# jyakaranda/A-LeGO-LOAM

Hardware: AMD Instinct MI355X
Metric: scans/sec (16x1800 LiDAR) full IP->LO->LM loop (higher is better)
Workload: dtype f32/f64

## Files before the change

### a-lego-loam_amd/csrc/alego_api.hip

```cpp
#include <hip/hip_runtime.h>

#include <cmath>
#include <cstdio>
#include <cstdlib>
#include <algorithm>
#include <cstring>
#include <mutex>
#include <set>
#include <string>
#include <vector>

#include "../../include/alego_mi355x.h"
#include "dev_common.h"
#include "dev_mem.h"
#include "front_end.h"
#include "lm_ctx.h"
#include "lm_host.h"
#include "merge_math.h"
#include "thin_math.h"
#include "loop_ctx.h"
#include "pgraph.h"
#include "prof.h"
#include "reloc.h"
#include "stream_plan.h"
// ... 769 lines not shown
    prev = m.stamp;
    const double qw = m.orientation[0], qx = m.orientation[1], qy = m.orientation[2], qz = m.orientation[3];
    double roll, pitch, yaw;
    {
      const double dd = qx * qx + qy * qy + qz * qz + qw * qw, sc = 2.0 / dd;
      const double xs = qx * sc, ys = qy * sc, zs = qz * sc;
      const double wx = qw * xs, wy = qw * ys, wz = qw * zs, xx = qx * xs, xy = qx * ys, xz = qx * zs, yy = qy * ys, yz = qy * zs, zz = qz * zs;
      const double m00 = 1.0 - (yy + zz), m10 = xy + wz, m20 = xz - wy, m21 = yz + wx, m22 = 1.0 - (xx + yy);
      if (std::fabs(m20) >= 1) {
        yaw = 0;
        const double delta = std::atan2(m21, m22);
        if (m20 < 0) { pitch = M_PI / 2.0; roll = delta; } else { pitch = -M_PI / 2.0; roll = delta; }
      } else {
        pitch = -std::asin(m20);
        roll = std::atan2(m21 / std::cos(pitch), m22 / std::cos(pitch));
        yaw = std::atan2(m10 / std::cos(pitch), m00 / std::cos(pitch));
      }
    }
    const double acc_x = m.linear_acceleration[0] + 9.81 * std::sin(pitch);
    const double acc_y = m.linear_acceleration[1] - 9.81 * std::cos(pitch) * std::sin(roll);
    const double acc_z = m.linear_acceleration[2] - 9.81 * std::cos(pitch) * std::cos(roll);
    const float w = (float)qw, x = (float)qx, y = (float)qy, z = (float)qz;
    const float tx = 2 * x, ty = 2 * y, tz = 2 * z;
    const float twx = tx * w, twy = ty * w, twz = tz * w, txx = tx * x, txy = ty * x, txz = tz * x, tyy = ty * y, tyz = tz * y, tzz = tz * z;
    const float R[3][3] = {{1 - (tyy + tzz), txy - twz, txz + twy}, {txy + twz, 1 - (txx + tzz), tyz - twx}, {txz - twy, tyz + twx, 1 - (txx + tyy)}};
    const float a[3] = {(float)acc_x, (float)acc_y, (float)acc_z};
    double* o = &pre[(size_t)i * 7];
    o[0] = m.stamp; o[1] = roll; o[2] = pitch; o[3] = yaw;
    for (int k = 0; k < 3; ++k) o[4 + k] = (double)(R[k][0] * a[0] + (R[k][1] * a[1] + R[k][2] * a[2]));
  }
  DevPool T;
  double* dp;
  HIP_TRY(h, T.get(&dp, pre.size(), false));
  hipStream_t S = stream_of(h, slot);
  HIP_TRY(h, hipMemcpyAsync(dp, pre.data(), pre.size() * 8, hipMemcpyHostToDevice, S));
  launch_lo_imu_push(h->d, slot, dp, n, S);
  HIP_TRY(h, hipStreamSynchronize(S));
  h->imu_last_stamp[slot] = prev;
  return 0;
}

int alego_profile_enable(alego_handle* h, int on) {
  if (!h) return ALEGO_ERR_ARG;
  hipSetDevice(h->device);
  HIP_TRY(h, sync_all(h));
  h->prof.reset();
  h->prof.on = on != 0;
  return 0;
}

int alego_profile_report(alego_handle* h, char* names, int names_cap, double* total_ms, int* launches, int cap) {
  if (!h) return ALEGO_ERR_ARG;
  hipSetDevice(h->device);
  HIP_TRY(h, sync_all(h));
  Profiler& P = h->prof;
  const int nk = (int)P.names.size();
  std::vector<double> tot(nk, 0.0);
  std::vector<int> cnt(nk, 0);
  for (auto& r : P.recs) {
    float ms = 0.f;
    if (hipEventElapsedTime(&ms, r.a, r.b) == hipSuccess) { tot[r.id] += ms; cnt[r.id]++; }
  }
  std::string joined;
  for (int i = 0; i < nk; ++i) { if (i) joined += ";"; joined += P.names[i]; }
  if ((int)joined.size() + 1 > names_cap || nk > cap) { h->err = "profile_report: buffers too small"; return ALEGO_ERR_CAPACITY; }
  std::memcpy(names, joined.c_str(), joined.size() + 1);
  for (int i = 0; i < nk; ++i) { total_ms[i] = tot[i]; launches[i] = cnt[i]; }
  return nk;
}

int alego_debug_voxel(alego_handle* h, const alego_point* pts, int n, float leaf, alego_point* out, int cap) {
  if (!h || n < 0 || (n > 0 && !pts)) return ALEGO_ERR_ARG;
  hipSetDevice(h->device);
  g_prof = &h->prof;
  DevPool T;
  float4 *din = nullptr, *dout = nullptr;
  int* cnt = nullptr;
  const int c = n > 0 ? n : 1;
  HIP_TRY(h, T.get(&din, (size_t)c, false)); HIP_TRY(h, T.get(&dout, (size_t)c, false)); HIP_TRY(h, T.get(&cnt, 2, false));
  const int hc[2] = {n, 0};
  HIP_TRY(h, hipMemcpy(cnt, hc, 8, hipMemcpyHostToDevice));
  if (n) HIP_TRY(h, hipMemcpy(din, pts, (size_t)n * 16, hipMemcpyHostToDevice));
  VoxJob job{din, cnt, dout, cnt + 1, nullptr, leaf, c, c, nullptr, 0};
  VoxCtx V;
  if (vox_create(&V, &job, 1, &h->err)) return ALEGO_ERR_HIP;
  int rc = vox_run(V, h->stream, &h->err);
  hipError_t e = hipStreamSynchronize(h->stream);
  int nout = 0;
  if (e == hipSuccess) e = hipMemcpy(&nout, cnt + 1, 4, hipMemcpyDeviceToHost);
  if (e == hipSuccess && rc == 0 && nout > cap) { h->err = "debug_voxel: output capacity"; rc = ALEGO_ERR_CAPACITY; }
  if (e == hipSuccess && rc == 0 && nout) e = hipMemcpy(out, dout, (size_t)nout * 16, hipMemcpyDeviceToHost);
  vox_destroy(&V);
  if (e != hipSuccess) { h->err = std::string("debug_voxel: ") + hipGetErrorString(e); return ALEGO_ERR_HIP; }
  return rc ? rc : nout;
}

int alego_debug_math(alego_handle* h, int mode, const float* a, const float* b, float* out, int n) {
  if (!h || n < 0 || mode < 0 || mode > 3 || (n > 0 && (!a || !out || (mode < 2 && !b)))) return ALEGO_ERR_ARG;
  if (n == 0) return 0;
  hipSetDevice(h->device);
  DevPool T;
  float *da, *db, *dout;
  HIP_TRY(h, T.get(&da, (size_t)n, false)); HIP_TRY(h, T.get(&db, (size_t)n, false)); HIP_TRY(h, T.get(&dout, (size_t)n, false));
  HIP_TRY(h, hipMemcpy(da, a, (size_t)n * 4, hipMemcpyHostToDevice));
  if (b) HIP_TRY(h, hipMemcpy(db, b, (size_t)n * 4, hipMemcpyHostToDevice));
  launch_atan2f_probe(da, db, dout, n, mode, h->stream);
  HIP_TRY(h, hipStreamSynchronize(h->stream));
  HIP_TRY(h, hipMemcpy(out, dout, (size_t)n * 4, hipMemcpyDeviceToHost));
  return 0;
}
int alego_debug_atan2f(alego_handle* h, const float* y, const float* x, float* out, int n) { return alego_debug_math(h, 0, y, x, out, n); }

int alego_debug_std_sort(alego_handle* h, const uint32_t* keys, int n, int depth_limit, int32_t* order) {
  if (!h || n < 0 || n > 4096 || (n > 0 && (!keys || !order))) return ALEGO_ERR_ARG;
  if (n == 0) return 0;
  hipSetDevice(h->device);
  DevPool T;
  uint32_t* dk;
  int* dp;
  HIP_TRY(h, T.get(&dk, (size_t)n, false)); HIP_TRY(h, T.get(&dp, (size_t)n, false));
  HIP_TRY(h, hipMemcpy(dk, keys, (size_t)n * 4, hipMemcpyHostToDevice));
  if (launch_stdsort_probe(dk, n, depth_limit, dp, h->stream)) return ALEGO_ERR_ARG;
  HIP_TRY(h, hipStreamSynchronize(h->stream));
  std::vector<int> pos(n), arr(n);
  HIP_TRY(h, hipMemcpy(pos.data(), dp, (size_t)n * 4, hipMemcpyDeviceToHost));
  for (int i = 0; i < n; ++i) { if (pos[i] < 0 || pos[i] >= n) { h->err = "alego_debug_std_sort: arrangement out of range"; return ALEGO_ERR_HIP; } arr[pos[i]] = i; }
  std::stable_sort(arr.begin(), arr.end(), [&](int a, int b) { return keys[a] < keys[b]; });
  for (int i = 0; i < n; ++i) order[i] = arr[i];
  return 0;
}

int alego_debug_eval_blocks(alego_handle* h, int type, int n, const double* geom13, const double* params6, double* res, double* jac6) {
  if (!h || n < 0 || type < 0 || type > 3 || !params6 || (n > 0 && (!geom13 || !res || !jac6))) return ALEGO_ERR_ARG;
  if (n == 0) return 0;
  hipSetDevice(h->device);
  DevPool T;
  double *dg, *dp, *dr, *dj;
  HIP_TRY(h, T.get(&dg, (size_t)n * 13, false)); HIP_TRY(h, T.get(&dp, 6, false)); HIP_TRY(h, T.get(&dr, (size_t)n, false)); HIP_TRY(h, T.get(&dj, (size_t)n * 6, false));
  HIP_TRY(h, hipMemcpy(dg, geom13, (size_t)n * 13 * 8, hipMemcpyHostToDevice));
  HIP_TRY(h, hipMemcpy(dp, params6, 48, hipMemcpyHostToDevice));
  launch_dbg_eval_blocks(type, n, dg, dp, dr, dj, h->stream);
  HIP_TRY(h, hipStreamSynchronize(h->stream));
  HIP_TRY(h, hipMemcpy(res, dr, (size_t)n * 8, hipMemcpyDeviceToHost));
  HIP_TRY(h, hipMemcpy(jac6, dj, (size_t)n * 48, hipMemcpyDeviceToHost));
  return 0;
}

int alego_debug_transform_to_start(alego_handle* h, const double* params6, const alego_point* pts, int n, alego_point* out) {
  if (!h || n < 0 || !params6 || (n > 0 && (!pts || !out))) return ALEGO_ERR_ARG;
  if (n == 0) return 0;
  hipSetDevice(h->device);
  DevPool T;
  double* dp;
  float4 *di, *dout;
  HIP_TRY(h, T.get(&dp, 6, false)); HIP_TRY(h, T.get(&di, (size_t)n, false)); HIP_TRY(h, T.get(&dout, (size_t)n, false));
  HIP_TRY(h, hipMemcpy(dp, params6, 48, hipMemcpyHostToDevice));
  HIP_TRY(h, hipMemcpy(di, pts, (size_t)n * 16, hipMemcpyHostToDevice));
  launch_dbg_transform_to_start(dp, di, n, dout, h->stream);
  HIP_TRY(h, hipStreamSynchronize(h->stream));
  HIP_TRY(h, hipMemcpy(out, dout, (size_t)n * 16, hipMemcpyDeviceToHost));
  return 0;
}

int alego_debug_check_guards(char* report, int cap) {
  std::string r;
  const int bad = guard_check(&r);
// ... 651 lines not shown
```

### a-lego-loam_amd/csrc/kernels_voxel.hip

```cpp
#include <algorithm>
#include <cstring>

#include <hip/hip_runtime.h>

#include <vector>

#include "voxel.h"
#include "wave.h"
#include "vgrid.h"
#include "dev_mem.h"
#include "prof.h"

typedef unsigned long long u64;

__device__ __forceinline__ bool vx_enabled(const VoxJob& J) { return J.enable == nullptr || *J.enable != 0; }

#ifndef VX_SMALL_MAX
#define VX_SMALL_MAX 8192
#endif

#ifndef VG_T
#define VG_T 512
#endif
#define VG_W (VG_T / 64)
// ... 154 lines not shown
  __threadfence_block();
  __syncthreads();
  VG_TICK(11);
  if (J.mode == 1) {
    for (int i = tid; i < min(n, J.out_cap); i += VG_T) outp[i] = J.in[(unsigned)srt[i]];
    if (tid == 0) { *J.n_out = min(n, J.out_cap); if (n > J.out_cap && J.overflow) *J.overflow = 1;
                    if (J.n_sel_out) J.n_sel_out[(size_t)sel * J.n_sel_stride] = min(n, J.out_cap); }
    __syncthreads();
    return;
  }
  auto head_rounds = [&](int r0, bool* head) {
    u64 cur[VG_U], prv[VG_U];
#pragma unroll
    for (int k = 0; k < VG_U; ++k) {
      const int i = r0 + 64 * k + lane;
      cur[k] = srt[min(i, n - 1)]; prv[k] = srt[max(min(i, n - 1) - 1, 0)];
    }
#pragma unroll
    for (int k = 0; k < VG_U; ++k) {
      const int i = r0 + 64 * k + lane;
      head[k] = i < seg1 && (i == 0 || (unsigned)(cur[k] >> 32) != (unsigned)(prv[k] >> 32));
    }
  };
  int* hl = reinterpret_cast<int*>(keys);
  int heads = 0;
  for (int r0 = seg0; r0 < seg1; r0 += 64 * VG_U) {
    bool head[VG_U];
    head_rounds(r0, head);
#pragma unroll
    for (int k = 0; k < VG_U; ++k) {
      const u64 hb = __ballot(head[k]);
      if (head[k]) hl[seg0 + heads + (int)__builtin_amdgcn_mbcnt_hi((unsigned)(hb >> 32), __builtin_amdgcn_mbcnt_lo((unsigned)hb, 0u))] = r0 + 64 * k + lane;
      heads += (int)__popcll(hb);
    }
  }
  if (lane == 0) s_w[wave] = heads;
  __threadfence_block();
  __syncthreads();
  if (tid == 0) {
    int run = 0;
    for (int w = 0; w < VG_W; ++w) { s_wbase[w] = run; run += s_w[w]; }
    s_wbase[VG_W] = run;
    int nf = n;
    s_nextfirst[VG_W] = n;
    for (int w = VG_W - 1; w >= 0; --w) { if (s_w[w] > 0) nf = hl[min(n, w * seglen)]; s_nextfirst[w] = nf; }
  }
  __syncthreads();
  const int nvox = s_wbase[VG_W];
  VG_TICK(12);
  for (int r = tid; r < min(nvox, J.out_cap); r += VG_T) {
    int w = 0;
#pragma unroll
    for (int q = 1; q < VG_W; ++q) w += (r >= s_wbase[q]) ? 1 : 0;
    const int loc = r - s_wbase[w], ws0 = min(n, w * seglen);
    const int a = hl[ws0 + loc], bn = hl[ws0 + min(loc + 1, s_w[w] - 1)];
    const int b = loc + 1 < s_w[w] ? bn : s_nextfirst[w + 1];
    float sx = 0.f, sy = 0.f, sz = 0.f, si = 0.f;
    for (int j = a; j < b; j += 8) {
      unsigned q[8];
      float4 pt[8];
#pragma unroll
      for (int k = 0; k < 8; ++k) q[k] = (unsigned)srt[min(j + k, b - 1)];
#pragma unroll
      for (int k = 0; k < 8; ++k) pt[k] = J.in[q[k]];
#pragma unroll
      for (int k = 0; k < 8; ++k) if (j + k < b) { sx += pt[k].x; sy += pt[k].y; sz += pt[k].z; si += pt[k].w; }
    }
    const float fn = (float)(b - a);
    J.out[r] = make_float4(sx / fn, sy / fn, sz / fn, si / fn);
  }
  if (tid == 0) { *J.n_out = min(nvox, J.out_cap); if (nvox > J.out_cap && J.overflow) *J.overflow = 1; }
  __syncthreads();
  VG_TICK(13);
}
#ifdef ALEGO_TIMING
extern "C" void alego_vg_times(long long* out) { (void)hipMemcpyFromSymbol(out, HIP_SYMBOL(vg_times), sizeof(long long) * 16); }
#endif

#define VX_SB 512
#define VS_W (VX_SB / 64)
#define VS_DMAX 9
#define VS_ND (1 << VS_DMAX)
__device__ __forceinline__ bool vx_less(const unsigned* key, unsigned a, unsigned b) { return key[a] < key[b] || (key[a] == key[b] && a < b); }

__device__ void vox_small_job(const VoxCtx& V, int job) {
  const VoxJob J = V.jobs[job];
  const int n = min(*J.n_in, J.cap);
  const int tid = threadIdx.x, lane = tid & 63, wave = tid >> 6;
  extern __shared__ __attribute__((aligned(16))) unsigned char vs_smem[];
  unsigned* s_key = reinterpret_cast<unsigned*>(vs_smem);
  unsigned short* s_ia = reinterpret_cast<unsigned short*>(vs_smem + 4 * VX_SMALL_MAX);
  unsigned short* s_ib = reinterpret_cast<unsigned short*>(vs_smem + 6 * VX_SMALL_MAX);
  unsigned short* s_cnt = reinterpret_cast<unsigned short*>(vs_smem + 8 * VX_SMALL_MAX);
  __shared__ float s_red[6][VX_SB / 64];
  __shared__ int s_scan[VX_SB / 64];
  __shared__ int s_tot[VS_ND];
  const int sel = (J.mode == 1 && J.out_sel) ? *J.out_sel : 0;
  float4* const outp = J.out + (size_t)sel * (J.mode == 1 ? J.out_stride : 0);
  if (n == 0) { if (tid == 0) { *J.n_out = 0; if (J.mode == 1 && J.n_sel_out) J.n_sel_out[(size_t)sel * J.n_sel_stride] = 0; } return; }
  const float inv = 1.0f / J.leaf;
  VG_TICK(0);
  float mn[3] = {3.402823466e+38f, 3.402823466e+38f, 3.402823466e+38f}, mx[3] = {-3.402823466e+38f, -3.402823466e+38f, -3.402823466e+38f};
  for (int i = tid; i < n; i += VX_SB) vgr_box_add(mn, mx, J.in[i]);
#pragma unroll
  for (int a = 0; a < 3; ++a) {
    bfly_minmax_f32(mn[a], mx[a]);
    if (lane == 0) { s_red[a][wave] = mn[a]; s_red[3 + a][wave] = mx[a]; }
  }
  __syncthreads();
#pragma unroll
  for (int a = 0; a < 3; ++a) {
    mn[a] = s_red[a][0]; mx[a] = s_red[3 + a][0];
#pragma unroll
    for (int w = 1; w < VX_SB / 64; ++w) { mn[a] = fminf(mn[a], s_red[a][w]); mx[a] = fmaxf(mx[a], s_red[3 + a][w]); }
  }
  if (tid < 3) {
    unsigned* bb = V.bbox + job * 8;
    bb[tid] = vgr_enc(tid == 0 ? mn[0] : tid == 1 ? mn[1] : mn[2]);
    bb[4 + tid] = ~vgr_enc(tid == 0 ? mx[0] : tid == 1 ? mx[1] : mx[2]);
  }
  if (J.mode == 1 && tid < 6 && J.box_out) J.box_out[(size_t)sel * 8 + (tid < 3 ? tid : tid + 1)] = tid == 0 ? mn[0] : tid == 1 ? mn[1] : tid == 2 ? mn[2] : tid == 3 ? mx[0] : tid == 4 ? mx[1] : mx[2];
  if (vgr_leaf_too_small(mn, mx, inv)) {
    for (int i = tid; i < min(n, J.out_cap); i += VX_SB) outp[i] = J.in[i];
    if (tid == 0) { *J.n_out = min(n, J.out_cap); if (n > J.out_cap && J.overflow) *J.overflow = 1;
                    if (J.mode == 1 && J.n_sel_out) J.n_sel_out[(size_t)sel * J.n_sel_stride] = min(n, J.out_cap); }
    return;
  }
  VG_TICK(1);
  const VgrGeom g = vgr_geom(mn, mx, inv);
  for (int i = tid; i < n; i += VX_SB) s_key[i] = vgr_id(g, J.in[i], inv);
  VG_TICK(2);
  const int bits = max(vgr_bits(g.T), 1);
  const int P = (bits + VS_DMAX - 1) / VS_DMAX, D = (bits + P - 1) / P, nd = 1 << D;
  const unsigned dmask = (unsigned)(nd - 1);
  const int seglen = ((n + VX_SB - 1) / VX_SB) * 64;
  const int seg0 = min(n, wave * seglen), seg1 = min(n, seg0 + seglen);
  unsigned short* my = s_cnt + wave * VS_ND;
  for (int p = 0; p < P; ++p) {
    const unsigned short* src = (p & 1) ? s_ia : s_ib;
    unsigned short* dst = (p & 1) ? s_ib : s_ia;
    const int sh = p * D;
    __syncthreads();
    for (int q = lane; q < nd; q += 64) my[q] = 0;
    for (int sweep = 0; sweep < 2; ++sweep) {
      if (sweep == 1) {
        __syncthreads();
        if (tid < nd) {
          int run = 0;
#pragma unroll
          for (int w = 0; w < VS_W; ++w) { const int c = s_cnt[w * VS_ND + tid]; s_cnt[w * VS_ND + tid] = (unsigned short)run; run += c; }
          s_tot[tid] = run;
        }
        __syncthreads();
        if (wave == 0) {
          constexpr int PER = VS_ND / 64;
          int v[PER], sum = 0;
#pragma unroll
          for (int k = 0; k < PER; ++k) { const int dgt = lane * PER + k; v[k] = dgt < nd ? s_tot[dgt] : 0; sum += v[k]; }
          const int incl = wave_incl_scan(sum);
          int run = incl - sum;
#pragma unroll
          for (int k = 0; k < PER; ++k) { const int dgt = lane * PER + k; if (dgt < nd) s_tot[dgt] = run; run += v[k]; }
        }
        __syncthreads();
      }
      for (int r0 = seg0; r0 < seg1; r0 += 64) {
        const int i = r0 + lane;
        const bool valid = i < seg1;
        const unsigned idx = valid ? (p == 0 ? (unsigned)i : (unsigned)src[i]) : 0u;
        const unsigned dg = valid ? (s_key[idx] >> sh) & dmask : 0u;
        unsigned long long m = __ballot(valid);
        for (int bit = 0; bit < D; ++bit) {
          const bool one = (dg >> bit) & 1u;
          const unsigned long long bal = __ballot(one);
          m &= one ? bal : ~bal;
        }
        const int rank = (int)__builtin_amdgcn_mbcnt_hi((unsigned)(m >> 32), __builtin_amdgcn_mbcnt_lo((unsigned)m, 0u));
        if (sweep == 1 && valid) dst[(int)my[dg] + s_tot[dg] + rank] = (unsigned short)idx;
        if (valid && rank == 0) my[dg] = (unsigned short)(my[dg] + (int)__popcll(m));
      }
    }
  }
  __syncthreads();
  const unsigned short* srt = (P & 1) ? s_ia : s_ib;
  unsigned short* hl = (P & 1) ? s_ib : s_ia;
  VG_TICK(3);
  if (J.mode == 1) {
    for (int i = tid; i < min(n, J.out_cap); i += VX_SB) outp[i] = J.in[srt[i]];
    if (tid == 0) { *J.n_out = min(n, J.out_cap); if (n > J.out_cap && J.overflow) *J.overflow = 1;
                    if (J.n_sel_out) J.n_sel_out[(size_t)sel * J.n_sel_stride] = min(n, J.out_cap); }
    __syncthreads();
    return;
  }
  int heads = 0;
  for (int r0 = seg0; r0 < seg1; r0 += 64) {
    const int i = r0 + lane;
    const bool head = i < seg1 && (i == 0 || s_key[srt[i]] != s_key[srt[i - 1]]);
    heads += (int)__popcll(__ballot(head));
  }
  if (lane == 0) s_scan[wave] = heads;
  __syncthreads();
  int vbase = 0, nvox = 0;
#pragma unroll
  for (int w = 0; w < VX_SB / 64; ++w) { const int c = s_scan[w]; if (w < wave) vbase += c; nvox += c; }
  for (int r0 = seg0; r0 < seg1; r0 += 64) {
    const int i = r0 + lane;
    const bool head = i < seg1 && (i == 0 || s_key[srt[i]] != s_key[srt[i - 1]]);
    const unsigned long long hb = __ballot(head);
    if (head) hl[vbase + (int)__builtin_amdgcn_mbcnt_hi((unsigned)(hb >> 32), __builtin_amdgcn_mbcnt_lo((unsigned)hb, 0u))] = (unsigned short)i;
    vbase += (int)__popcll(hb);
  }
  __syncthreads();
  VG_TICK(4);
  VG_TICK(5);
  VG_TICK(6);
  for (int r = tid; r < min(nvox, J.out_cap); r += VX_SB) {
    const int a = hl[r], b = r + 1 < nvox ? (int)hl[r + 1] : n;
    float sx = 0.f, sy = 0.f, sz = 0.f, si = 0.f;
    for (int j = a; j < b; j += 4) {
      float4 pt[4];
#pragma unroll
      for (int k = 0; k < 4; ++k) pt[k] = J.in[srt[min(j + k, b - 1)]];
#pragma unroll
      for (int k = 0; k < 4; ++k) if (j + k < b) { sx += pt[k].x; sy += pt[k].y; sz += pt[k].z; si += pt[k].w; }
    }
    const float fn = (float)(b - a);
    J.out[r] = make_float4(sx / fn, sy / fn, sz / fn, si / fn);
  }
  if (tid == 0) { *J.n_out = min(nvox, J.out_cap); if (nvox > J.out_cap && J.overflow) *J.overflow = 1; }
  __syncthreads();
  VG_TICK(7);
}
__global__ void __launch_bounds__(VX_SB) vox_small(VoxCtx V) {
  extern __shared__ __attribute__((aligned(16))) unsigned char vs_smem_k[];
  const int cnt = V.cnt[0];
  for (int j = blockIdx.x; j < cnt; j += gridDim.x) {
    vox_small_job(V, V.list_small[j]);
    __syncthreads();
  }
  const int nbig = V.cnt[1];
  if ((int)blockIdx.x < V.grid_big) {
    for (int j = blockIdx.x; j < nbig; j += min((int)gridDim.x, V.grid_big)) {
      vox_big_job(V, V.list_big[j], vs_smem_k);
      __syncthreads();
    }
  }
}

__global__ void __launch_bounds__(256) vox_plan(VoxCtx V) {
  __shared__ int s_n[2];
  if (threadIdx.x < 2) s_n[threadIdx.x] = 0;
  __syncthreads();
  for (int j = threadIdx.x; j < V.njobs; j += 256) {
    const VoxJob J = V.jobs[j];
    if (!vx_enabled(J)) continue;
    const int n = min(*J.n_in, J.cap);
    if (n == 0) { *J.n_out = 0; if (J.mode == 1 && J.n_sel_out) J.n_sel_out[(size_t)(J.out_sel ? *J.out_sel : 0) * J.n_sel_stride] = 0; continue; }
    if (n <= VX_SMALL_MAX) V.list_small[atomicAdd(&s_n[0], 1)] = j;
    else V.list_big[atomicAdd(&s_n[1], 1)] = j;
  }
  __syncthreads();
  if (threadIdx.x < 2) V.cnt[threadIdx.x] = s_n[threadIdx.x];
}

#define VX_SMALL_LDS (8 * VX_SMALL_MAX + 2 * VS_W * VS_ND)
int vox_create(VoxCtx* V, const VoxJob* jobs, int njobs, std::string* err) {
  std::memset(V, 0, sizeof(*V));
  if (hipFuncSetAttribute(reinterpret_cast<const void*>(vox_small), hipFuncAttributeMaxDynamicSharedMemorySize, VX_SMALL_LDS) != hipSuccess) { *err = "vox_create: hipFuncSetAttribute"; return -2; }
// ... 36 lines not shown
```

### a-lego-loam_amd/csrc/lm_host.hip

```cpp
#include "lm_host.h"
#include "dev_mem.h"

#include <cstdio>
#include <cstdlib>
#include <algorithm>
#include <cstring>
#include <vector>

#include <rccl/rccl.h>

#include "kf_store.h"
#include "voxel.h"
#include "gmap.h"
#include "loc_math.h"
#include "pgraph.h"
#include "merge.h"
#include "merge_math.h"
#include "thin.h"
#include "thin_math.h"

struct LmHost {
  alego_params P;
  int n_slots;
  int gsize;
// ... 46 lines not shown
  int* li = L.li + (size_t)slot * LI_COUNT;
  for (int m = 0; m < 2; ++m) {
    const int cap = m ? L.total_cap : L.kf_cap_c;
    VoxJob j{(m ? L.kf_tmp_s : L.kf_tmp_c) + (size_t)slot * cap, li + LI_TMPN_C + m, (m ? L.kfs_s : L.kfs_c) + kf_row_at(L, slot, 0) * cap, li + LI_SORT_N + m, li + LI_KF_PENDING,
             m ? P.lm_leaf_surf : P.lm_leaf_corner, cap, cap, li + LI_OVERFLOW, 0};
    j.mode = 1; j.out_sel = li + LI_KF_PEND_RING; j.out_stride = cap;
    j.box_out = L.kfs_box + kf_run_at(L, slot, m, 0) * 8; j.n_sel_out = L.kfs_n + kf_run_at(L, slot, m, 0); j.n_sel_stride = 1;
    out->push_back(j);
  }
}
}

LmHost* lm_host_create(const alego_params& P, const DevCtx& d, int n_slots, int gsize, const std::vector<hipStream_t>& st, std::string* err) {
  LmHost* lm = new LmHost();
  lm->P = P; lm->n_slots = n_slots; lm->gsize = gsize; lm->st = st; lm->frames.assign(n_slots, 0);
  lm->gv.small_max = gv_small_max_env();
  VoxCtx vz; std::memset(&vz, 0, sizeof(VoxCtx));
  lm->vm.assign(st.size(), vz); lm->v2.assign(st.size(), vz); lm->vk.assign(st.size(), vz);
  lm->work.assign(st.size(), MapWork{nullptr, nullptr, 0});
  LmCtx& L = lm->L;
  std::memset(&L, 0, sizeof(L));
  L.K = P.recent_keyframe_num > 0 ? P.recent_keyframe_num : 1;
  L.KR = L.K + 1;
  L.fr_stride = L.KR; L.fr_mod = L.KR;
  lm->fallback_ok = n_slots <= 64 || !d.opt_map_merge;
  L.in_cap_c = d.fcap[F_LSHARP]; L.in_cap_s = d.N; L.in_cap_o = d.N;
  L.kf_cap_c = d.fcap[F_LSHARP];
  L.kf_cap_s = P.kf_cap_surf > 0 ? std::min(P.kf_cap_surf, d.N) : d.N / 2;
  L.kf_cap_o = P.kf_cap_outlier > 0 ? std::min(P.kf_cap_outlier, d.N) : d.N / 4;
  L.kf_cap_s = std::max(L.kf_cap_s, L.kf_cap_c - L.kf_cap_o);
  L.total_cap = L.kf_cap_s + L.kf_cap_o;
  L.map_cap_c = L.K * L.kf_cap_c; L.map_cap_s = L.K * L.total_cap;
  L.gcap = n_slots <= 64 ? (1 << 20) : (1 << 18);
  L.qcap = L.kf_cap_c + L.total_cap;
  {
    const size_t mx = lm_solve_row_bytes_max();
    const char* e = getenv("ALEGO_LM_ROW_LDS");
    int dev = 0, cus = 256;
    if (hipGetDevice(&dev) != hipSuccess || hipDeviceGetAttribute(&cus, hipDeviceAttributeMultiprocessorCount, dev) != hipSuccess) cus = 256;
    const size_t dflt = gsize > cus ? (size_t)72 * 1024 : lm_solve_row_bytes_default();
    L.solve_row_bytes = (int)(e ? std::min(mx, (size_t)std::max(0, atoi(e))) : std::min(mx, dflt));
  }
  const size_t B = n_slots;
  bool ok = true;
  ok = ok && A(lm, &L.li, B * LI_COUNT, err) && A(lm, &L.ld, B * LD_COUNT, err);
  ok = ok && A(lm, &L.stage_odom, B * 2 * 8, err);
  ok = ok && A(lm, &L.in_corner, B * L.in_cap_c, err) && A(lm, &L.in_surf, B * L.in_cap_s, err) && A(lm, &L.in_outl, B * L.in_cap_o, err);
  ok = ok && ring_alloc(lm, L, B * L.KR, err);
  ok = ok && A(lm, &L.kf_tmp_c, B * L.kf_cap_c, err) && A(lm, &L.kf_tmp_s, B * L.total_cap, err);
  ok = ok && A(lm, &L.rec, B * L.K, err) && A(lm, &L.rec_prev, B * L.K, err);
  ok = ok && A(lm, &L.U_c, B * L.map_cap_c, err) && A(lm, &L.U_s, B * L.map_cap_s, err) && A(lm, &L.Ucnt_c, B * L.map_cap_c, err) && A(lm, &L.Ucnt_s, B * L.map_cap_s, err);
  ok = ok && A(lm, &L.newkeys, B * 2 * L.total_cap, err) && A(lm, &L.map_bbox, B * 2 * 8, err);
  {
    double* part = nullptr; int* ctl = nullptr; double* state = nullptr;
    ok = ok && A(lm, &part, B * 32, err) && A(lm, &ctl, B * 8, err) && A(lm, &state, B * 64, err);
    L.shard_part = part; L.shard_ctl = ctl; L.shard_state = state;
  }
  ok = ok && A(lm, &L.map_corner_raw, lm->fallback_ok ? B * L.map_cap_c : 1, err) && A(lm, &L.map_surf_raw, lm->fallback_ok ? B * L.map_cap_s : 1, err);
  ok = ok && A(lm, &L.map_corner_ds, B * L.map_cap_c, err) && A(lm, &L.map_surf_ds, B * L.map_cap_s, err);
  ok = ok && A(lm, &L.cur_corner_ds, B * L.kf_cap_c, err) && A(lm, &L.cur_surf_ds, B * L.kf_cap_s, err) && A(lm, &L.cur_outl_ds, B * L.kf_cap_o, err);
  ok = ok && A(lm, &L.cur_total, B * L.total_cap, err) && A(lm, &L.cur_total_ds, B * L.total_cap, err);
  ok = ok && A(lm, &L.grid, B * 2, err) && A(lm, &L.cell_start, B * 2 * ((size_t)L.gcap + 1), err) && A(lm, &L.cell_cur, B * 2 * ((size_t)L.gcap + 1), err);
  ok = ok && A(lm, &L.cell_pts, B * 2 * L.map_cap_s, err);
  ok = ok && A(lm, &L.blocks, B * L.qcap * 8, err) && A(lm, &L.crows, B * L.qcap * 10, err) && A(lm, &L.knn, B * L.qcap * 5, err);
  if (!ok) { lm_host_destroy(lm); return nullptr; }
  std::vector<double> ld(B * LD_COUNT, 0.0);
  for (size_t b = 0; b < B; ++b) { ld[b * LD_COUNT + LD_Q_M2O] = 1.0; ld[b * LD_COUNT + LD_Q_O2L] = 1.0; ld[b * LD_COUNT + LD_Q_M2L] = 1.0; }
  if (hipMemcpy(L.ld, ld.data(), ld.size() * sizeof(double), hipMemcpyHostToDevice) != hipSuccess) { *err = "lm_host_create: upload failed"; lm_host_destroy(lm); return nullptr; }
  std::vector<int> li0(B * LI_COUNT, 0);
  for (size_t b = 0; b < B; ++b) li0[b * LI_COUNT + LI_LATEST] = -1;
  if (hipMemcpy(L.li, li0.data(), li0.size() * sizeof(int), hipMemcpyHostToDevice) != hipSuccess) { *err = "lm_host_create: upload failed"; lm_host_destroy(lm); return nullptr; }
  for (size_t g = 0; g < st.size(); ++g) {
  std::vector<VoxJob> jm, j1, j2, jk;
  for (size_t b = g * gsize; b < B && b < (g + 1) * (size_t)gsize; ++b) {
    int* li = L.li + b * LI_COUNT;
    if (lm->fallback_ok) {
      jm.push_back(VoxJob{L.map_corner_raw + b * L.map_cap_c, li + LI_KRAW_C, L.map_corner_ds + b * L.map_cap_c, li + LI_KDS_C, li + LI_REBUILD_FB, P.lm_leaf_corner, L.map_cap_c, L.map_cap_c, li + LI_OVERFLOW, 0});
      jm.push_back(VoxJob{L.map_surf_raw + b * L.map_cap_s, li + LI_KRAW_S, L.map_surf_ds + b * L.map_cap_s, li + LI_KDS_S, li + LI_REBUILD_FB, P.lm_leaf_surf, L.map_cap_s, L.map_cap_s, li + LI_OVERFLOW, 0});
    }
    j1.push_back(VoxJob{L.in_corner + b * L.in_cap_c, li + LI_NIN_C, L.cur_corner_ds + b * L.kf_cap_c, li + LI_NCUR_C, li + LI_RUN, P.lm_leaf_corner, L.in_cap_c, L.kf_cap_c, li + LI_OVERFLOW, 0});
    j1.push_back(VoxJob{L.in_surf + b * L.in_cap_s, li + LI_NIN_S, L.cur_surf_ds + b * L.kf_cap_s, li + LI_NCUR_S, li + LI_RUN, P.lm_leaf_surf, L.in_cap_s, L.kf_cap_s, li + LI_OVERFLOW, 0});
    j1.push_back(VoxJob{L.in_outl + b * L.in_cap_o, li + LI_NIN_O, L.cur_outl_ds + b * L.kf_cap_o, li + LI_NCUR_O, li + LI_RUN, P.lm_leaf_outlier, L.in_cap_o, L.kf_cap_o, li + LI_OVERFLOW, 0});
    j2.push_back(VoxJob{L.cur_total + b * L.total_cap, li + LI_NTOTAL, L.cur_total_ds + b * L.total_cap, li + LI_NTOTAL_DS, li + LI_RUN, P.lm_leaf_surf, L.total_cap, L.total_cap, li + LI_OVERFLOW, 0});
    kf_sort_jobs(L, P, (int)b, &jk);
  }
  const int ns = (int)j1.size() / 3;
  jm.insert(jm.end(), j1.begin(), j1.end());
  jm.insert(jm.end(), jk.begin(), jk.end());
  if (vox_create(&lm->vm[g], jm.data(), (int)jm.size(), err) || vox_create(&lm->v2[g], j2.data(), (int)j2.size(), err) ||
      vox_create(&lm->vk[g], jk.data(), (int)jk.size(), err)) { lm_host_destroy(lm); return nullptr; }
  const bool big_scans = d.N > 8 * 8192;
  lm->vm[g].grid_small = 3 * ns + std::max(2, ns / 2);
  if (const char* e = getenv("ALEGO_VOX_GRID_DIV")) { const int dv = std::max(1, atoi(e)); lm->vm[g].grid_small = std::max(2, lm->vm[g].grid_small / dv); lm->v2[g].grid_small = std::max(1, lm->v2[g].grid_small / dv); }
  lm->vm[g].grid_big = (!d.opt_map_merge || big_scans) ? std::max(2, ns / 2) : std::min(8, std::max(2, ns / 2));
  lm->v2[g].grid_big = big_scans ? std::max(2, ns / 2) : std::max(1, ns / 16);
  lm->vk[g].grid_small = 2; lm->vk[g].grid_big = 2;
  MapWork& W = lm->work[g];
  W.cap = std::max(4096, 64 * ns);
  if (!A(lm, &W.items, (size_t)W.cap, err) || !A(lm, &W.count, 2, err)) { lm_host_destroy(lm); return nullptr; }
  }
  return lm;
}

void lm_host_destroy(LmHost* lm) {
  if (!lm) return;
  if (lm->comm) { (void)ncclCommDestroy(lm->comm); lm->comm = nullptr; }
  for (auto& v : lm->vm) vox_destroy(&v);
  for (auto& v : lm->v2) vox_destroy(&v);
  for (auto& v : lm->vk) vox_destroy(&v);
  if (lm->vloc_made) vox_destroy(&lm->vloc);
  gv_destroy(&lm->gv);
  lm->mg_pairs.clear(); lm->mg_items.clear(); lm->mg_tail.clear(); lm->mg_moves.clear();
  lm->th_jobs.clear(); lm->th_ints.clear(); lm->th_prot.clear(); lm->th_items.clear(); lm->th_pts.clear(); lm->th_rows.clear(); lm->th_pose.clear();
  lm->mem.clear();
  delete lm;
}

static bool dbg_sync(hipStream_t st, const char* what, std::string* err) {
  static const bool on = getenv("ALEGO_DEBUG_SYNC") != nullptr;
  if (!on) return true;
  hipError_t e = hipStreamSynchronize(st);
  if (e == hipSuccess) e = hipGetLastError();
  fprintf(stderr, "[alego dbg] %s: %s\n", what, hipGetErrorString(e));
  if (e != hipSuccess) { *err = std::string(what) + ": " + hipGetErrorString(e); return false; }
  return true;
}

static int map_sequence(LmHost* lm, const DevCtx& d, const LmCtx& L, int g, hipStream_t st, std::string* err) {
  if (!d.opt_map_merge) {
    if (!lm->fallback_ok) { *err = "ALEGO_MAP_MERGE=0 needs the handle to be created with it (more than 64 slots)"; return ALEGO_ERR_ARG; }
    launch_lm_concat(d, L, st);
    if (!dbg_sync(st, "lm_concat", err)) return ALEGO_ERR_HIP;
  }
  if (int r = vox_run(lm->vm[g], st, err)) return r;
  if (!dbg_sync(st, "vox round 1", err)) return ALEGO_ERR_HIP;
  launch_map_update(d, L, lm->work[g], st);
  if (!dbg_sync(st, "map_update", err)) return ALEGO_ERR_HIP;
  if (d.opt_map_merge) {
    launch_map_accum(d, L, lm->work[g], st);
    if (!dbg_sync(st, "map_accum", err)) return ALEGO_ERR_HIP;
  }
  launch_lm_grid(d, L, st);
  if (!dbg_sync(st, "lm_grid", err)) return ALEGO_ERR_HIP;
  return 0;
}

static int lm_allreduce(void* ctx, double* buf, size_t count, hipStream_t st) {
  LmHost* lm = static_cast<LmHost*>(ctx);
  const ncclResult_t r = ncclAllReduce(buf, buf, count, ncclDouble, ncclSum, lm->comm, st);
  if (r != ncclSuccess) { lm->dist_err = std::string("ncclAllReduce: ") + ncclGetErrorString(r); return ALEGO_ERR_HIP; }
  return 0;
}

struct LmAsync { hipStream_t front, back; hipEvent_t staged, back_same, back_other; long k; };
static int lm_sequence(LmHost* lm, const DevCtx& d, int stage, const std::vector<char>& odom_valid, std::string* err, hipStream_t st_override = nullptr, const LmAsync* A = nullptr) {
  const int g = d.slot0 / lm->gsize;
  hipStream_t st = A ? A->back : (st_override ? st_override : lm->st[g]);
  LmCtx L = lm->L;
  L.vox_bbox = lm->vm[g].bbox; L.vox_slot0 = g * lm->gsize;
  int n_run = 0, n_norun = 0;
  for (int i = 0; i < d.n_launch; ++i) {
    long& f = lm->frames[d.slot0 + i];
    const bool run = odom_valid[i] && (f % lm->P.lm_every) == 0;
    if (odom_valid[i]) ++f;
    run ? ++n_run : ++n_norun;
  }
// ... 826 lines not shown
```

### a-lego-loam_amd/csrc/voxel.h

```cpp
#ifndef ALEGO_VOXEL_H_
#define ALEGO_VOXEL_H_
#include <hip/hip_runtime.h>

#include <string>

struct VoxJob {
  const float4* in;
  const int* n_in;
  float4* out;
  int* n_out;
  const int* enable;
  float leaf;
  int cap;
  int out_cap;
  int* overflow;
  int off;
  int mode;
  const int* out_sel;
  int out_stride;
  float* box_out;
  int* n_sel_out;
  int n_sel_stride;
};

struct VoxCtx {
  VoxJob* jobs;
  int njobs;
  unsigned* bbox;
  unsigned* keys;
  unsigned long long *pairs_a, *pairs_b;
  int *list_small, *list_big, *cnt;
  int grid_small, grid_big;
  unsigned total;
};

int vox_create(VoxCtx* V, const VoxJob* jobs, int njobs, std::string* err);
void vox_destroy(VoxCtx* V);
int vox_run(const VoxCtx& V, hipStream_t st, std::string* err);

#endif
```

Before: 472,500.

## Add tiny-job wave path, presorted merge fast path, and atomic digit counting to voxel sort

Jobs with 64 or fewer points are handled by a single wavefront that ranks keys through readlane comparisons instead of a radix sort. For jobs flagged as presorted (the concatenated total cloud), the kernel counts descents and, when the keys are already sorted or form two sorted runs or a short unsorted tail, builds the permutation by binary-search merging and skips the radix passes. The radix histogram pass now uses packed 16-bit shared-memory atomics instead of the earlier counting loop. These paths add branches and a pass to detect descents, and the atomic counting may contend on heavily repeated digits.

```diff
diff --git a/a-lego-loam_amd/csrc/alego_api.hip b/a-lego-loam_amd/csrc/alego_api.hip
--- a/a-lego-loam_amd/csrc/alego_api.hip
+++ b/a-lego-loam_amd/csrc/alego_api.hip
@@ -875,6 +875,7 @@
   HIP_TRY(h, hipMemcpy(cnt, hc, 8, hipMemcpyHostToDevice));
   if (n) HIP_TRY(h, hipMemcpy(din, pts, (size_t)n * 16, hipMemcpyHostToDevice));
   VoxJob job{din, cnt, dout, cnt + 1, nullptr, leaf, c, c, nullptr, 0};
+  job.presorted_hint = 1;
   VoxCtx V;
   if (vox_create(&V, &job, 1, &h->err)) return ALEGO_ERR_HIP;
   int rc = vox_run(V, h->stream, &h->err);
diff --git a/a-lego-loam_amd/csrc/kernels_voxel.hip b/a-lego-loam_amd/csrc/kernels_voxel.hip
--- a/a-lego-loam_amd/csrc/kernels_voxel.hip
+++ b/a-lego-loam_amd/csrc/kernels_voxel.hip
@@ -260,6 +260,101 @@
 #define VS_DMAX 9
 #define VS_ND (1 << VS_DMAX)
 __device__ __forceinline__ bool vx_less(const unsigned* key, unsigned a, unsigned b) { return key[a] < key[b] || (key[a] == key[b] && a < b); }
+#ifndef VX_CNT_ATOMIC
+#define VX_CNT_ATOMIC 1
+#endif
+#ifndef VX_TINY
+#define VX_TINY 1
+#endif
+#ifndef VX_MERGE
+#define VX_MERGE 1
+#endif
+static_assert(VX_SMALL_MAX % VX_SB == 0 && VX_SMALL_MAX / VX_SB * 64 < 65536, "a wavefront's segment must fit a 16-bit digit counter");
+__device__ __forceinline__ void vx_wave_sync() {
+  __builtin_amdgcn_fence(__ATOMIC_RELEASE, "wavefront");
+  __builtin_amdgcn_wave_barrier();
+  __builtin_amdgcn_fence(__ATOMIC_ACQUIRE, "wavefront");
+}
+__device__ __forceinline__ int vx_count_below(const unsigned* k, int lo, int hi, unsigned key, bool or_equal) {
+  int a = lo, e = hi;
+  while (a < e) {
+    const int m = (a + e) >> 1;
+    const unsigned v = k[m];
+    if (or_equal ? v <= key : v < key) a = m + 1; else e = m;
+  }
+  return a - lo;
+}
+
+#if VX_TINY
+__device__ void vox_tiny_job(const VoxCtx& V, int job, const VoxJob& J, int n, unsigned* s_key, unsigned short* srt, unsigned short* hl) {
+  const int lane = threadIdx.x;
+  const bool valid = lane < n;
+  const int sel = (J.mode == 1 && J.out_sel) ? *J.out_sel : 0;
+  float4* const outp = J.out + (size_t)sel * (J.mode == 1 ? J.out_stride : 0);
+  const float inv = 1.0f / J.leaf;
+  VG_TICK(0);
+  float mn[3] = {3.402823466e+38f, 3.402823466e+38f, 3.402823466e+38f}, mx[3] = {-3.402823466e+38f, -3.402823466e+38f, -3.402823466e+38f};
+  const float4 pt = J.in[min(lane, n - 1)];
+  if (valid) vgr_box_add(mn, mx, pt);
+#pragma unroll
+  for (int a = 0; a < 3; ++a) bfly_minmax_f32(mn[a], mx[a]);
+  if (lane < 3) {
+    unsigned* bb = V.bbox + job * 8;
+    bb[lane] = vgr_enc(lane == 0 ? mn[0] : lane == 1 ? mn[1] : mn[2]);
+    bb[4 + lane] = ~vgr_enc(lane == 0 ? mx[0] : lane == 1 ? mx[1] : mx[2]);
+  }
+  if (J.mode == 1 && lane < 6 && J.box_out) J.box_out[(size_t)sel * 8 + (lane < 3 ? lane : lane + 1)] = lane == 0 ? mn[0] : lane == 1 ? mn[1] : lane == 2 ? mn[2] : lane == 3 ? mx[0] : lane == 4 ? mx[1] : mx[2];
+  if (vgr_leaf_too_small(mn, mx, inv)) {
+    if (lane < min(n, J.out_cap)) outp[lane] = pt;
+    if (lane == 0) { *J.n_out = min(n, J.out_cap); if (n > J.out_cap && J.overflow) *J.overflow = 1;
+                     if (J.mode == 1 && J.n_sel_out) J.n_sel_out[(size_t)sel * J.n_sel_stride] = min(n, J.out_cap); }
+    return;
+  }
+  VG_TICK(1);
+  const VgrGeom g = vgr_geom(mn, mx, inv);
+  const unsigned key = vgr_id(g, pt, inv);
+  if (valid) s_key[lane] = key;
+  VG_TICK(2);
+  int rank = 0;
+  for (int j = 0; j < n; ++j) {
+    const unsigned kj = (unsigned)__builtin_amdgcn_readlane((int)key, j);
+    rank += (kj < key || (kj == key && j < lane)) ? 1 : 0;
+  }
+  if (valid) srt[rank] = (unsigned short)lane;
+  vx_wave_sync();
+  VG_TICK(3);
+  if (J.mode == 1) {
+    if (lane < min(n, J.out_cap)) outp[lane] = J.in[srt[lane]];
+    if (lane == 0) { *J.n_out = min(n, J.out_cap); if (n > J.out_cap && J.overflow) *J.overflow = 1;
+                     if (J.n_sel_out) J.n_sel_out[(size_t)sel * J.n_sel_stride] = min(n, J.out_cap); }
+    return;
+  }
+  const bool head = valid && (lane == 0 || s_key[srt[lane]] != s_key[srt[lane - 1]]);
+  const unsigned long long hb = __ballot(head);
+  const int nvox = (int)__popcll(hb);
+  if (head) hl[(int)__builtin_amdgcn_mbcnt_hi((unsigned)(hb >> 32), __builtin_amdgcn_mbcnt_lo((unsigned)hb, 0u))] = (unsigned short)lane;
+  vx_wave_sync();
+  VG_TICK(4);
+  VG_TICK(5);
+  VG_TICK(6);
+  if (lane < min(nvox, J.out_cap)) {
+    const int r = lane;
+    const int a = hl[r], b = r + 1 < nvox ? (int)hl[r + 1] : n;
+    float sx = 0.f, sy = 0.f, sz = 0.f, si = 0.f;
+    for (int j = a; j < b; j += 4) {
+      float4 q[4];
+#pragma unroll
+      for (int k = 0; k < 4; ++k) q[k] = J.in[srt[min(j + k, b - 1)]];
+#pragma unroll
+      for (int k = 0; k < 4; ++k) if (j + k < b) { sx += q[k].x; sy += q[k].y; sz += q[k].z; si += q[k].w; }
+    }
+    const float fn = (float)(b - a);
+    J.out[r] = make_float4(sx / fn, sy / fn, sz / fn, si / fn);
+  }
+  if (lane == 0) { *J.n_out = min(nvox, J.out_cap); if (nvox > J.out_cap && J.overflow) *J.overflow = 1; }
+  VG_TICK(7);
+}
+#endif
 
 __device__ void vox_small_job(const VoxCtx& V, int job) {
   const VoxJob J = V.jobs[job];
@@ -273,9 +368,18 @@
   __shared__ float s_red[6][VX_SB / 64];
   __shared__ int s_scan[VX_SB / 64];
   __shared__ int s_tot[VS_ND];
+#if VX_MERGE
+  __shared__ int s_desc[2];
+#endif
   const int sel = (J.mode == 1 && J.out_sel) ? *J.out_sel : 0;
   float4* const outp = J.out + (size_t)sel * (J.mode == 1 ? J.out_stride : 0);
   if (n == 0) { if (tid == 0) { *J.n_out = 0; if (J.mode == 1 && J.n_sel_out) J.n_sel_out[(size_t)sel * J.n_sel_stride] = 0; } return; }
+#if VX_TINY
+  if (n <= 64) {
+    if (wave == 0) vox_tiny_job(V, job, J, n, s_key, s_ia, s_ib);
+    return;
+  }
+#endif
   const float inv = 1.0f / J.leaf;
   VG_TICK(0);
   float mn[3] = {3.402823466e+38f, 3.402823466e+38f, 3.402823466e+38f}, mx[3] = {-3.402823466e+38f, -3.402823466e+38f, -3.402823466e+38f};
@@ -306,15 +410,53 @@
   }
   VG_TICK(1);
   const VgrGeom g = vgr_geom(mn, mx, inv);
+#if VX_MERGE
+  if (J.presorted_hint && tid < 2) s_desc[tid] = tid ? n : 0;
+#endif
   for (int i = tid; i < n; i += VX_SB) s_key[i] = vgr_id(g, J.in[i], inv);
   VG_TICK(2);
+  bool sorted = false;
+#if VX_MERGE
+  if (J.presorted_hint) {
+    __syncthreads();
+    for (int i0 = 0; i0 < n; i0 += VX_SB) {
+      const int i = i0 + tid;
+      const unsigned long long db = __ballot(i > 0 && i < n && s_key[min(i, n - 1)] < s_key[max(min(i, n - 1) - 1, 0)]);
+      if (db != 0 && lane == 0) { atomicAdd(&s_desc[0], (int)__popcll(db)); atomicMin(&s_desc[1], i0 + wave * 64 + (int)__ffsll(db) - 1); }
+    }
+    __syncthreads();
+    const int ndesc = s_desc[0], b = min(s_desc[1], n), m = n - b;
+    if (ndesc == 0) {
+      sorted = true;
+      for (int i = tid; i < n; i += VX_SB) s_ia[i] = (unsigned short)i;
+    } else if (m <= 64) {
+      sorted = true;
+      unsigned* s_tk = reinterpret_cast<unsigned*>(s_tot);
+      if (wave == 0) {
+        const unsigned kt = s_key[b + min(lane, m - 1)];
+        int r = 0;
+        for (int j = 0; j < m; ++j) {
+          const unsigned kj = (unsigned)__builtin_amdgcn_readlane((int)kt, j);
+          r += (kj < kt || (kj == kt && j < lane)) ? 1 : 0;
+        }
+        if (lane < m) { s_tk[r] = kt; s_ia[r + vx_count_below(s_key, 0, b, kt, true)] = (unsigned short)(b + lane); }
+      }
+      __syncthreads();
+      for (int i = tid; i < b; i += VX_SB) s_ia[i + vx_count_below(s_tk, 0, m, s_key[i], false)] = (unsigned short)i;
+    } else if (ndesc == 1) {
+      sorted = true;
+      for (int i = tid; i < n; i += VX_SB)
+        s_ia[i < b ? i + vx_count_below(s_key, b, n, s_key[i], false) : (i - b) + vx_count_below(s_key, 0, b, s_key[i], true)] = (unsigned short)i;
+    }
+  }
+#endif
   const int bits = max(vgr_bits(g.T), 1);
   const int P = (bits + VS_DMAX - 1) / VS_DMAX, D = (bits + P - 1) / P, nd = 1 << D;
   const unsigned dmask = (unsigned)(nd - 1);
   const int seglen = ((n + VX_SB - 1) / VX_SB) * 64;
   const int seg0 = min(n, wave * seglen), seg1 = min(n, seg0 + seglen);
   unsigned short* my = s_cnt + wave * VS_ND;
-  for (int p = 0; p < P; ++p) {
+  for (int p = 0; p < (sorted ? 0 : P); ++p) {
     const unsigned short* src = (p & 1) ? s_ia : s_ib;
     unsigned short* dst = (p & 1) ? s_ib : s_ia;
     const int sh = p * D;
@@ -342,6 +484,16 @@
         }
         __syncthreads();
       }
+#if VX_CNT_ATOMIC
+      if (sweep == 0) {
+        unsigned* myw = reinterpret_cast<unsigned*>(my);
+        for (int i = seg0 + lane; i < seg1; i += 64) {
+          const unsigned dg = (s_key[p == 0 ? (unsigned)i : (unsigned)src[i]] >> sh) & dmask;
+          atomicAdd(&myw[dg >> 1], 1u << (16 * (dg & 1u)));
+        }
+        continue;
+      }
+#endif
       for (int r0 = seg0; r0 < seg1; r0 += 64) {
         const int i = r0 + lane;
         const bool valid = i < seg1;
@@ -360,8 +512,9 @@
     }
   }
   __syncthreads();
-  const unsigned short* srt = (P & 1) ? s_ia : s_ib;
-  unsigned short* hl = (P & 1) ? s_ib : s_ia;
+  const bool in_a = sorted || (P & 1);
+  const unsigned short* srt = in_a ? s_ia : s_ib;
+  unsigned short* hl = in_a ? s_ib : s_ia;
   VG_TICK(3);
   if (J.mode == 1) {
     for (int i = tid; i < min(n, J.out_cap); i += VX_SB) outp[i] = J.in[srt[i]];
diff --git a/a-lego-loam_amd/csrc/lm_host.hip b/a-lego-loam_amd/csrc/lm_host.hip
--- a/a-lego-loam_amd/csrc/lm_host.hip
+++ b/a-lego-loam_amd/csrc/lm_host.hip
@@ -152,6 +152,7 @@
     j1.push_back(VoxJob{L.in_surf + b * L.in_cap_s, li + LI_NIN_S, L.cur_surf_ds + b * L.kf_cap_s, li + LI_NCUR_S, li + LI_RUN, P.lm_leaf_surf, L.in_cap_s, L.kf_cap_s, li + LI_OVERFLOW, 0});
     j1.push_back(VoxJob{L.in_outl + b * L.in_cap_o, li + LI_NIN_O, L.cur_outl_ds + b * L.kf_cap_o, li + LI_NCUR_O, li + LI_RUN, P.lm_leaf_outlier, L.in_cap_o, L.kf_cap_o, li + LI_OVERFLOW, 0});
     j2.push_back(VoxJob{L.cur_total + b * L.total_cap, li + LI_NTOTAL, L.cur_total_ds + b * L.total_cap, li + LI_NTOTAL_DS, li + LI_RUN, P.lm_leaf_surf, L.total_cap, L.total_cap, li + LI_OVERFLOW, 0});
+    j2.back().presorted_hint = 1;
     kf_sort_jobs(L, P, (int)b, &jk);
   }
   const int ns = (int)j1.size() / 3;
diff --git a/a-lego-loam_amd/csrc/voxel.h b/a-lego-loam_amd/csrc/voxel.h
--- a/a-lego-loam_amd/csrc/voxel.h
+++ b/a-lego-loam_amd/csrc/voxel.h
@@ -21,6 +21,7 @@
   float* box_out;
   int* n_sel_out;
   int n_sel_stride;
+  int presorted_hint;
 };
 
 struct VoxCtx {
```

Result: no change. 477,000 (median of 6 runs) (+1.0%).
